# sshaoshuai/PointRCNN

Hardware: AMD Instinct MI355X
Metric: KITTI frames/sec, RPN inference end-to-end (16384 pts/frame, bs32 per GPU) (higher is better)
Workload: dtype f32 via split-bf16x6 MFMA (every fp32 operand cut exactly into 3 bf16 pieces, 6 bf16 MFMA products per fp32 product, fp32 accumulate: fp32-grade, measured error 2.9e-7 of sum|x||w| vs 3.0e-7 for the fp32-MFMA kernel; hoisted grouped layers on the split kernel too, unhoisted grouped first layers (xyz; 1 GPU; Full RPN PointNet++ backbone (4 SA-MSG + 4 FP) + cls/reg heads, tools/cfgs/default.yaml, 16384 pts/frame, batch 32 per GPU, random-init weights, eval-mode BN; frames_per_gpu=32, npoints=16384, parallelism=frames sharded, dp1, launch=hipGraph replay, streams=20, hw_queues=4, proposal_layer=normal, clouds=uniform, group_dedup=True, roi_dedup=True

## Files before the change

### pointrcnn_amd/csrc/fps.hip

```cpp
#include "lds_sort.h"
#include "switches.h"

typedef float f32x2 __attribute__((ext_vector_type(2)));
template <int PPT> struct fvec_t { typedef float type __attribute__((ext_vector_type(PPT))); };
template <> struct fvec_t<1> { typedef float type __attribute__((ext_vector_type(2))); };

#define FPS_DPP_MAX(v, ctrl) asm volatile("s_nop 1\n\tv_max_i32_dpp %0, %0, %0 " ctrl : "+v"(v))

__device__ __forceinline__ int wave_max_i32_fused(int v) {
    FPS_DPP_MAX(v, "row_shr:1 row_mask:0xf bank_mask:0xf");
    FPS_DPP_MAX(v, "row_shr:2 row_mask:0xf bank_mask:0xf");
    FPS_DPP_MAX(v, "row_shr:4 row_mask:0xf bank_mask:0xf");
    FPS_DPP_MAX(v, "row_shr:8 row_mask:0xf bank_mask:0xf");
    FPS_DPP_MAX(v, "row_bcast:15 row_mask:0xa bank_mask:0xf");
    FPS_DPP_MAX(v, "row_bcast:31 row_mask:0xc bank_mask:0xf");
    asm volatile("s_nop 1");
    return __builtin_amdgcn_readlane(v, 63);
}
__device__ __forceinline__ int row0_max_i32_fused(int v) {
    FPS_DPP_MAX(v, "row_shr:1 row_mask:0xf bank_mask:0xf");
    FPS_DPP_MAX(v, "row_shr:2 row_mask:0xf bank_mask:0xf");
    FPS_DPP_MAX(v, "row_shr:4 row_mask:0xf bank_mask:0xf");
    FPS_DPP_MAX(v, "row_shr:8 row_mask:0xf bank_mask:0xf");
    asm volatile("s_nop 1");
// ... 125 lines not shown
        int k = tid * PPT + i;
        bool ok = k < N;
        px[i] = ok ? p[k * 3 + 0] : 0.f;
        py[i] = ok ? p[k * 3 + 1] : 0.f;
        pz[i] = ok ? p[k * 3 + 2] : 0.f;
        pt[i] = ok ? 1e10f : -1.0f;
    }
    if (tid == 0 && npoint > 0) out[0] = 0;
    float x0 = p[0], y0 = p[1], z0 = p[2];

    for (int j = 1; j < npoint; j++) {
        float best = -2.0f;
        if (PPT >= 2) {
            const f32x2 qx = {x0, x0}, qy = {y0, y0}, qz = {z0, z0};
#pragma unroll
            for (int i = 0; i + 1 < PPT; i += 2) {
                f32x2 dx = (f32x2){px[i], px[i + 1]} - qx;
                f32x2 dy = (f32x2){py[i], py[i + 1]} - qy;
                f32x2 dz = (f32x2){pz[i], pz[i + 1]} - qz;
                f32x2 d = (dx * dx + dy * dy) + dz * dz;
                float t0 = __builtin_fminf(pt[i], d.x), t1 = __builtin_fminf(pt[i + 1], d.y);
                pt[i] = t0; pt[i + 1] = t1;
                best = __builtin_fmaxf(best, __builtin_fmaxf(t0, t1));
            }
        } else {
            float d = sqdist3(px[0], py[0], pz[0], x0, y0, z0);
            float t = __builtin_fminf(pt[0], d);
            pt[0] = t;
            best = t;
        }
        const int wmax = wave_max_i32_fused(__float_as_int(best));
        const float wmaxf = __int_as_float(wmax);
        const int owner = __builtin_ctzll(__ballot(best == wmaxf));
        int myslot = PPT - 1;
#pragma unroll
        for (int i = PPT - 2; i >= 0; i--) myslot = (pt[i] == best) ? i : myslot;
        const int istar = __builtin_amdgcn_readlane(myslot, owner);
        const int widx = (wave * 64 + owner) * PPT + istar;
        float sx = px[istar], sy = py[istar], sz = pz[istar];
        float wx = __int_as_float(__builtin_amdgcn_readlane(__float_as_int(sx), owner));
        float wy = __int_as_float(__builtin_amdgcn_readlane(__float_as_int(sy), owner));
        float wz = __int_as_float(__builtin_amdgcn_readlane(__float_as_int(sz), owner));
        int gidx;
        if (NW == 1) {
            gidx = widx; x0 = wx; y0 = wy; z0 = wz;
        } else {
            float* s = slot[j & 1][wave];
            if (lane == 0) {
                s[0] = wmaxf; s[1] = __int_as_float(widx);
                s[2] = wx; s[3] = wy; s[4] = wz;
            }
            __syncthreads();
            const float* r = slot[j & 1][lane < NW ? lane : 0];
            int v = lane < NW ? __float_as_int(r[0]) : (int)0x80000000;
            int id = __float_as_int(r[1]);
            float rx = r[2], ry = r[3], rz = r[4];
            const int gmax = row0_max_i32_fused(v);
            const int wwin = __builtin_ctzll(__ballot(v == gmax));
            gidx = __builtin_amdgcn_readlane(id, wwin);
            x0 = __int_as_float(__builtin_amdgcn_readlane(__float_as_int(rx), wwin));
            y0 = __int_as_float(__builtin_amdgcn_readlane(__float_as_int(ry), wwin));
            z0 = __int_as_float(__builtin_amdgcn_readlane(__float_as_int(rz), wwin));
        }
        if (tid == 0) out[j] = gidx;
    }
}

#define FPS_BIG 1.0e18f
#ifndef FPS_V
#define FPS_V 6
#endif
#ifndef FPS_PAIR_ASM
#define FPS_PAIR_ASM 1
#endif

__device__ __forceinline__ unsigned morton_spread6(unsigned v) {
    v &= 0x3fu;
    v = (v | (v << 8)) & 0x0000300fu;
    v = (v | (v << 4)) & 0x000030c3u;
    v = (v | (v << 2)) & 0x00009249u;
    return v;
}

__global__ __launch_bounds__(1024) void fps_sort_kernel(const float* __restrict__ xyz, int N, int NP, int32_t* __restrict__ perm,
                                                        const int32_t* __restrict__ skip) {
    if (skip && skip[blockIdx.x]) return;
    extern __shared__ unsigned keys[];
    __shared__ float red[6][16];
    const int b = blockIdx.x, tid = threadIdx.x, lane = tid & 63, wave = tid >> 6, nw = blockDim.x >> 6;
    const float* __restrict__ p = xyz + (size_t)b * N * 3;
    float lo[3] = {FPS_BIG, FPS_BIG, FPS_BIG}, hi[3] = {-FPS_BIG, -FPS_BIG, -FPS_BIG};
    for (int k = tid; k < N; k += blockDim.x)
#pragma unroll
        for (int a = 0; a < 3; a++) { float v = p[k * 3 + a]; lo[a] = fminf(lo[a], v); hi[a] = fmaxf(hi[a], v); }
#pragma unroll
    for (int a = 0; a < 3; a++) {
        for (int o = 32; o > 0; o >>= 1) { lo[a] = fminf(lo[a], __shfl_xor(lo[a], o)); hi[a] = fmaxf(hi[a], __shfl_xor(hi[a], o)); }
        if (lane == 0) { red[a][wave] = lo[a]; red[3 + a][wave] = hi[a]; }
    }
    __syncthreads();
    float scale[3];
#pragma unroll
    for (int a = 0; a < 3; a++) {
        float l = red[a][0], h = red[3 + a][0];
        for (int w = 1; w < nw; w++) { l = fminf(l, red[a][w]); h = fmaxf(h, red[3 + a][w]); }
        lo[a] = l;
        scale[a] = (h > l) ? 63.0f / (h - l) : 0.f;
    }
    unsigned v[16];
    if (tid * 16 < NP) {
#pragma unroll
        for (int e = 0; e < 16; e++) {
            const int k = tid * 16 + e;
            unsigned key = ~0u;
            if (k < N) {
                unsigned qx = (unsigned)((p[k * 3 + 0] - lo[0]) * scale[0]);
                unsigned qy = (unsigned)((p[k * 3 + 1] - lo[1]) * scale[1]);
                unsigned qz = (unsigned)((p[k * 3 + 2] - lo[2]) * scale[2]);
                unsigned m = (morton_spread6(qx) << 2) | (morton_spread6(qz) << 1) | morton_spread6(qy);
                key = (m << 14) | (unsigned)k;
            }
            v[e] = key;
        }
    }
    block_sort16(v, keys, NP, tid);
    if (tid * 16 < NP) {
#pragma unroll
        for (int e = 0; e < 16; e++) {
            const int k = tid * 16 + e;
            if (k < N) perm[(size_t)b * N + k] = (int32_t)(v[e] & 0x3fffu);
        }
    }
}

#define FPS_DPP_MIN(v, ctrl) asm volatile("s_nop 1\n\tv_min_i32_dpp %0, %0, %0 " ctrl : "+v"(v))
#define FPS_DPP_FMIN(v, ctrl) asm volatile("s_nop 1\n\tv_min_f32_dpp %0, %0, %0 " ctrl : "+v"(v))
#define FPS_DPP_FMAX(v, ctrl) asm volatile("s_nop 1\n\tv_max_f32_dpp %0, %0, %0 " ctrl : "+v"(v))
#define FPS_WAVE_REDUCE(MACRO, v)                                   \
    MACRO(v, "row_shr:1 row_mask:0xf bank_mask:0xf");               \
    MACRO(v, "row_shr:2 row_mask:0xf bank_mask:0xf");               \
    MACRO(v, "row_shr:4 row_mask:0xf bank_mask:0xf");               \
    MACRO(v, "row_shr:8 row_mask:0xf bank_mask:0xf");               \
    MACRO(v, "row_bcast:15 row_mask:0xa bank_mask:0xf");            \
    MACRO(v, "row_bcast:31 row_mask:0xc bank_mask:0xf");            \
    asm volatile("s_nop 1");

__device__ __forceinline__ int wave_min_i32_fused(int v) { FPS_WAVE_REDUCE(FPS_DPP_MIN, v) return __builtin_amdgcn_readlane(v, 63); }
__device__ __forceinline__ float wave_min_f32_fused(float v) {
    FPS_WAVE_REDUCE(FPS_DPP_FMIN, v) return __int_as_float(__builtin_amdgcn_readlane(__float_as_int(v), 63));
}
__device__ __forceinline__ float wave_max_f32_fused(float v) {
    FPS_WAVE_REDUCE(FPS_DPP_FMAX, v) return __int_as_float(__builtin_amdgcn_readlane(__float_as_int(v), 63));
}
__device__ __forceinline__ int row0_min_i32_fused(int v) {
    FPS_DPP_MIN(v, "row_shr:1 row_mask:0xf bank_mask:0xf");
    FPS_DPP_MIN(v, "row_shr:2 row_mask:0xf bank_mask:0xf");
    FPS_DPP_MIN(v, "row_shr:4 row_mask:0xf bank_mask:0xf");
    FPS_DPP_MIN(v, "row_shr:8 row_mask:0xf bank_mask:0xf");
    asm volatile("s_nop 1");
    return __builtin_amdgcn_readlane(v, 15);
}

#define FPS_XT_DECL __shared__ __attribute__((aligned(256))) unsigned xt[3][64]
struct fps_cand_t { float x, y, z; unsigned long long key; };
__device__ __forceinline__ void fps_cand_set(fps_cand_t& c, int wave, float cx, float cy, float cz, float cval, int corig) {
    const unsigned hi = (unsigned)__float_as_int(cval) ^ 0x80000000u;
    const unsigned lo = ((0xFFFFFFFu - (unsigned)min(corig, 0xFFFFFFF)) << 4) | (unsigned)wave;
    c.x = cx; c.y = cy; c.z = cz; c.key = ((unsigned long long)hi << 32) | lo;
    asm volatile("" : "+v"(c.x), "+v"(c.y), "+v"(c.z), "+v"(c.key));
}
__device__ __forceinline__ void fps_xt_publish(unsigned (*xt)[64], int cb, int wave, const fps_cand_t& c) {
    unsigned* t = xt[cb];
    t[wave] = __float_as_uint(c.x); t[16 + wave] = __float_as_uint(c.y); t[32 + wave] = __float_as_uint(c.z);
    asm volatile("ds_max_u64 %0, %1 offset:192" : : "v"((unsigned)(size_t)&t[0]), "v"(c.key) : "memory");
    if (wave == 0) *(unsigned long long*)&xt[cb == 2 ? 0 : cb + 1][48] = 0ULL;
}
__device__ __forceinline__ int fps_xt_collect(unsigned (*xt)[64], int cb, int lane, float& x0, float& y0, float& z0, int& wl) {
    const int tv = (int)xt[cb][lane];
    const unsigned klo = (unsigned)__builtin_amdgcn_readlane(tv, 48);
    wl = (int)(klo & 15u);
    x0 = __int_as_float(__builtin_amdgcn_readlane(tv, wl));
    y0 = __int_as_float(__builtin_amdgcn_readlane(tv, wl | 16));
    z0 = __int_as_float(__builtin_amdgcn_readlane(tv, wl | 32));
    return (int)(0xFFFFFFFu - (klo >> 4));
}

#ifdef PRCNN_FPS_TIMING
__device__ unsigned long long prcnn_fps_dbg[16 * 8 + 16 + 16 * 16];
PRCNN_API int prcnn_fps_timing_read(unsigned long long* host_out) {
    return hipMemcpyFromSymbol(host_out, HIP_SYMBOL(prcnn_fps_dbg), sizeof(prcnn_fps_dbg)) == hipSuccess ? 0 : -1;
}
#define FPS_T(...) __VA_ARGS__
#ifndef PRCNN_FPS_TIMING_WAVE
#define PRCNN_FPS_TIMING_WAVE -1
#endif
#define FPS_NOW(w) ((PRCNN_FPS_TIMING_WAVE < 0 || (w) == PRCNN_FPS_TIMING_WAVE) ? __builtin_readcyclecounter() : 0ULL)
#else
#define FPS_T(...)
#endif

template <int PPT>
__global__ __launch_bounds__(1024) void fps_pruned_kernel(const float* __restrict__ xyz, const int32_t* __restrict__ perm,
                                                          int N, int npoint, int32_t* __restrict__ idx_out, const int32_t* __restrict__ skip) {
    if (skip && skip[blockIdx.x]) return;
    constexpr int BLOCK = 1024, NW = 16;
    typedef typename fvec_t<PPT>::type fvec;
    FPS_XT_DECL;
    extern __shared__ int s_po[];
// ... 669 lines not shown

__global__ __launch_bounds__(1024) void fps_mem_kernel(const float* __restrict__ xyz, int N, int npoint,
                                                       float* __restrict__ tmp, int32_t* __restrict__ idx_out) {
    constexpr int NW = 16;
    __shared__ int sval[2][NW], sidx[2][NW];
    const int b = blockIdx.x, tid = threadIdx.x, lane = tid & 63, wave = tid >> 6;
    const float* __restrict__ p = xyz + (size_t)b * N * 3;
    float* __restrict__ t = tmp + (size_t)b * N;
    int32_t* __restrict__ out = idx_out + (size_t)b * npoint;
    for (int k = tid; k < N; k += 1024) t[k] = 1e10f;
    if (tid == 0 && npoint > 0) out[0] = 0;
    int old = 0;
    for (int j = 1; j < npoint; j++) {
        float x0 = p[old * 3], y0 = p[old * 3 + 1], z0 = p[old * 3 + 2];
        float best = -2.0f;
        int bk = 0x7fffffff;
        for (int k = tid; k < N; k += 1024) {
            float d = sqdist3(p[k * 3], p[k * 3 + 1], p[k * 3 + 2], x0, y0, z0);
            float v = t[k];
            v = d < v ? d : v;
            t[k] = v;
            if (v > best) { best = v; bk = k; }
        }
        int vb = __float_as_int(best);
        int wmax = wave_max_i32(vb);
        int widx = wave_min_i32(vb == wmax ? bk : 0x7fffffff);
        if (lane == 0) { sval[j & 1][wave] = wmax; sidx[j & 1][wave] = widx; }
        __syncthreads();
        int v = lane < NW ? sval[j & 1][lane] : (int)0x80000000;
        int id = lane < NW ? sidx[j & 1][lane] : 0x7fffffff;
        int gmax = row0_max_i32(v);
        old = row0_min_i32(v == gmax ? id : 0x7fffffff);
        if (tid == 0) out[j] = old;
    }
}

template <int BLOCK, int PPT>
static void launch_fps(const float* xyz, int B, int N, int npoint, int32_t* idx, const int32_t* skip, hipStream_t s) {
    hipLaunchKernelGGL((fps_reg_kernel<BLOCK, PPT>), dim3(B), dim3(BLOCK), 0, s, xyz, N, npoint, idx, skip);
}

static int* fps_timeout_word() {
    static int* word = [] {
        int* w = nullptr;
        if (hipHostMalloc((void**)&w, sizeof(int), hipHostMallocMapped) != hipSuccess) { (void)hipGetLastError(); return (int*)nullptr; }
        *w = 0;
        return w;
    }();
    return word;
}

PRCNN_API int prcnn_fps_status(void) {
    int* w = fps_timeout_word();
    if (w && __atomic_exchange_n(w, 0, __ATOMIC_RELAXED) != 0)
        return prcnn_fail(PRCNN_EHIP, "prcnn_fps: a multi-workgroup launch (N > 16384) gave up waiting for a partner slice; "
                                      "its output holds -1 indices (were all ceil(N/16384) workgroups of a frame able to become resident?)");
    return PRCNN_OK;
}

__global__ __launch_bounds__(256) void fps_prefix_kernel(const float* __restrict__ xyz, const int32_t* __restrict__ prev_idx, int N, int npoint,
                                                         int32_t* __restrict__ idx_out, int32_t* __restrict__ skip) {
    const int b = blockIdx.x, tid = threadIdx.x;
    const float* __restrict__ p = xyz + (size_t)b * N * 3;
    const int32_t* __restrict__ pi = prev_idx + (size_t)b * N;
    int32_t* __restrict__ out = idx_out + (size_t)b * npoint;
    bool ok = true;
    for (int k = tid; k < 3 * N; k += 256) ok &= fabsf(p[k]) < 1e4f;
    for (int j = 1 + tid; j < npoint; j += 256) ok &= pi[j] != 0;
    const int pass = __syncthreads_and(ok) ? 1 : 0;
    if (pass)
        for (int j = tid; j < npoint; j += 256) out[j] = j;
    if (tid == 0) skip[b] = pass;
}

static int fps_dispatch(const float* xyz, int B, int N, int npoint, float* tmp, int32_t* idx, const int32_t* skip, hipStream_t s) {
    if (tmp && N > 2048 && N <= 16384) {
        int NP = 1;
        while (NP < N) NP <<= 1;
        int32_t* perm = reinterpret_cast<int32_t*>(tmp);
        static PrcnnLdsLimit sort_attr;
        if (!sort_attr.raise((const void*)fps_sort_kernel, 80 * 1024))
            return prcnn_fail(PRCNN_EHIP, "prcnn_fps: cannot raise the dynamic LDS limit of the sort kernel");
        const int sort_threads = NP / 16 < 64 ? 64 : NP / 16;
        hipLaunchKernelGGL(fps_sort_kernel, dim3(B), dim3(sort_threads), lds_sort_bytes(NP, sizeof(unsigned)), s, xyz, N, NP, perm, skip);
        PRCNN_LAUNCH_CHECK("prcnn_fps(sort)");
        static PrcnnLdsLimit pruned_attr;
        if (!pruned_attr.raise((const void*)fps_pruned_kernel<16>, 16 * 4096))
            return prcnn_fail(PRCNN_EHIP, "prcnn_fps: cannot raise the dynamic LDS limit of the pruned kernel");
        const bool slots = sw_enabled(SW_FPS_SLOTS);
        static PrcnnLdsLimit slot_attr;
        if (slots && N > 8192 && !slot_attr.raise((const void*)fps_slot_kernel<16, 16>, 16 * 4096))
            return prcnn_fail(PRCNN_EHIP, "prcnn_fps: cannot raise the dynamic LDS limit of the slot kernel");
        const bool batch = sw_opt_in(SW_FPS_BATCH);
        static PrcnnLdsLimit batch_attr;
        if (slots && batch && N > 8192 && !batch_attr.raise((const void*)fps_batch_kernel<16, 16>, 16 * 4096))
            return prcnn_fail(PRCNN_EHIP, "prcnn_fps: cannot raise the dynamic LDS limit of the batch kernel");
        if (slots && batch && N > 8192) hipLaunchKernelGGL((fps_batch_kernel<16, 16>), dim3(B), dim3(1024), 16 * 4096, s, xyz, perm, N, npoint, idx, skip);
        else if (slots && N > 8192) hipLaunchKernelGGL((fps_slot_kernel<16, 16>), dim3(B), dim3(1024), 16 * 4096, s, xyz, perm, N, npoint, idx, skip);
        else if (N <= 4096) hipLaunchKernelGGL((fps_pruned_kernel<4>), dim3(B), dim3(1024), 4 * 4096, s, xyz, perm, N, npoint, idx, skip);
        else if (N <= 8192) hipLaunchKernelGGL((fps_pruned_kernel<8>), dim3(B), dim3(1024), 8 * 4096, s, xyz, perm, N, npoint, idx, skip);
        else hipLaunchKernelGGL((fps_pruned_kernel<16>), dim3(B), dim3(1024), 16 * 4096, s, xyz, perm, N, npoint, idx, skip);
    }
    else if (N <= 64) launch_fps<64, 1>(xyz, B, N, npoint, idx, skip, s);
    else if (N <= 128) launch_fps<64, 2>(xyz, B, N, npoint, idx, skip, s);
    else if (N <= 256) launch_fps<64, 4>(xyz, B, N, npoint, idx, skip, s);
    else if (N <= 512) launch_fps<64, 8>(xyz, B, N, npoint, idx, skip, s);
    else if (N <= 1024) launch_fps<64, 16>(xyz, B, N, npoint, idx, skip, s);
    else if (N <= 2048) launch_fps<256, 8>(xyz, B, N, npoint, idx, skip, s);
    else if (N <= 4096) launch_fps<256, 16>(xyz, B, N, npoint, idx, skip, s);
    else if (N <= 8192) launch_fps<1024, 8>(xyz, B, N, npoint, idx, skip, s);
    else if (N <= 16384) launch_fps<1024, 16>(xyz, B, N, npoint, idx, skip, s);
    else {
        PRCNN_REQUIRE(tmp, "prcnn_fps: N=%d > 16384 needs the (B,N) tmp buffer", N);
        PRCNN_REQUIRE(!skip, "prcnn_fps: the multi-workgroup kernels (N=%d > 16384) take no skip words", N);
        const int S = prcnn_divup(N, FPS_MULTI_SLICE);
        const bool use_mem = sw_present(SW_FPS_MEM);
        if (!use_mem && S <= FPS_MULTI_MAX_SPLIT && ((uintptr_t)tmp & 7) == 0) {
            const size_t slot_bytes = (size_t)B * 2 * S * 5 * sizeof(unsigned long long);
            if (prcnn_fill_words(tmp, 0xFFFFFFFFu, slot_bytes / 4, s) != hipSuccess) return prcnn_fail(PRCNN_EHIP, "prcnn_fps: cannot clear the exchange slots");
            if (int st = prcnn_fps_status()) return st;
            hipLaunchKernelGGL(fps_multi_kernel, dim3(B * S), dim3(1024), 0, s, xyz, N, npoint, S, reinterpret_cast<unsigned long long*>(tmp), idx,
                               fps_timeout_word());
        } else {
            hipLaunchKernelGGL(fps_mem_kernel, dim3(B), dim3(1024), 0, s, xyz, N, npoint, tmp, idx);
        }
    }
    PRCNN_LAUNCH_CHECK("prcnn_fps");
    return PRCNN_OK;
}

PRCNN_API int prcnn_fps(const float* xyz, int B, int N, int npoint, float* tmp, int32_t* idx, prcnn_stream_t stream) {
    PRCNN_REQUIRE(B >= 0 && N > 0 && npoint >= 0, "prcnn_fps: bad shape B=%d N=%d npoint=%d", B, N, npoint);
    PRCNN_REQUIRE(npoint <= N, "prcnn_fps: npoint %d > N %d", npoint, N);
    if (B == 0 || npoint == 0) return PRCNN_OK;
    PRCNN_REQUIRE(xyz && idx, "prcnn_fps: null pointer");
    return fps_dispatch(xyz, B, N, npoint, tmp, idx, nullptr, (hipStream_t)stream);
}

PRCNN_API int prcnn_fps_nested(const float* xyz, const int32_t* prev_idx, int B, int N, int npoint, float* tmp, int32_t* idx, int32_t* skip,
                               prcnn_stream_t stream) {
    PRCNN_REQUIRE(B >= 0 && N > 0 && npoint >= 0, "prcnn_fps_nested: bad shape B=%d N=%d npoint=%d", B, N, npoint);
    PRCNN_REQUIRE(npoint <= N, "prcnn_fps_nested: npoint %d > N %d", npoint, N);
    PRCNN_REQUIRE(N <= 16384, "prcnn_fps_nested: N=%d > 16384 (call prcnn_fps)", N);
    if (B == 0 || npoint == 0) return PRCNN_OK;
    PRCNN_REQUIRE(xyz && prev_idx && idx && skip, "prcnn_fps_nested: null pointer");
    hipStream_t s = (hipStream_t)stream;
    hipLaunchKernelGGL(fps_prefix_kernel, dim3(B), dim3(256), 0, s, xyz, prev_idx, N, npoint, idx, skip);
    PRCNN_LAUNCH_CHECK("prcnn_fps_nested(prefix)");
    return fps_dispatch(xyz, B, N, npoint, tmp, idx, skip, s);
}

__global__ __launch_bounds__(1024) void fps_upstream_order_kernel(const float* __restrict__ xyz, int N, int npoint, int T,
                                                                  float* __restrict__ tmp, int32_t* __restrict__ idx_out) {
    constexpr int NWMAX = 16;
    __shared__ int sval[2][NWMAX], stid[2][NWMAX], sidx[2][NWMAX];
    const int b = blockIdx.x, tid = threadIdx.x, lane = tid & 63, wave = tid >> 6;
    const int nw = (blockDim.x + 63) >> 6;
    const float* __restrict__ p = xyz + (size_t)b * N * 3;
    float* __restrict__ t = tmp + (size_t)b * N;
    int32_t* __restrict__ out = idx_out + (size_t)b * npoint;
    for (int k = tid; k < N; k += blockDim.x) t[k] = 1e10f;
    if (tid == 0 && npoint > 0) out[0] = 0;
    __syncthreads();
    int old = 0;
    for (int j = 1; j < npoint; j++) {
        const float x0 = p[old * 3], y0 = p[old * 3 + 1], z0 = p[old * 3 + 2];
        float best = -2.0f;
// ... 41 lines not shown
```

### pointrcnn_amd/csrc/lds_sort.h

```cpp
#pragma once
#include "common.h"

typedef unsigned long long u64;

__device__ __forceinline__ int lds_phys(int i) { return i + (i >> 4); }

template <class K>
__device__ __forceinline__ void cswap(K& a, K& b, bool up) {
    const bool gt = a > b;
    if (gt == up) { K t = a; a = b; b = t; }
}

template <class K>
__device__ __forceinline__ void merge16(K (&v)[16], bool up) {
#pragma unroll
    for (int j = 8; j >= 1; j >>= 1)
#pragma unroll
        for (int e = 0; e < 16; e++)
            if ((e & j) == 0) cswap(v[e], v[e | j], up);
}

template <class K>
__device__ __forceinline__ void lds_pass(K* keys, int nact, int t, int j, int k) {
    K a[8], c[8];
    if (j <= nact && nact >= 8) {
        const int i0 = ((t & ~(j - 1)) << 1) | (t & (j - 1));
        const int D = 2 * nact, DP = D + (D >> 4);
        K* pa = keys + lds_phys(i0);
        K* pb = keys + lds_phys(i0 + j);
#pragma unroll
        for (int q = 0; q < 8; q++) { a[q] = pa[q * DP]; c[q] = pb[q * DP]; }
#pragma unroll
        for (int q = 0; q < 8; q++) {
            const bool up = ((i0 + q * D) & k) == 0;
            if ((a[q] > c[q]) == up) { pa[q * DP] = c[q]; pb[q * DP] = a[q]; }
        }
    } else {
        int ia[8];
#pragma unroll
        for (int q = 0; q < 8; q++) {
            const int p = q * nact + t;
            ia[q] = ((p & ~(j - 1)) << 1) | (p & (j - 1));
            a[q] = keys[lds_phys(ia[q])]; c[q] = keys[lds_phys(ia[q] + j)];
        }
#pragma unroll
        for (int q = 0; q < 8; q++) {
            const bool up = (ia[q] & k) == 0;
            if ((a[q] > c[q]) == up) { keys[lds_phys(ia[q])] = c[q]; keys[lds_phys(ia[q] + j)] = a[q]; }
        }
    }
}

static inline size_t lds_sort_bytes(int Npad, size_t key_bytes = sizeof(u64)) { return ((size_t)(Npad + (Npad >> 4)) + 1) * key_bytes; }

template <class K>
__device__ __forceinline__ void block_sort16(K (&v)[16], K* keys, int Npad, int t) {
    const int nact = Npad >> 4;
    const bool active = t < nact;
    if (active) {
#pragma unroll
        for (int k = 2; k <= 16; k <<= 1)
#pragma unroll
            for (int j = k >> 1; j >= 1; j >>= 1)
#pragma unroll
                for (int e = 0; e < 16; e++)
                    if ((e & j) == 0) cswap(v[e], v[e | j], k < 16 ? ((e & k) == 0) : ((t & 1) == 0));
#pragma unroll
        for (int e = 0; e < 16; e++) keys[lds_phys(t * 16 + e)] = v[e];
    }
    __syncthreads();
    for (int k = 32; k <= Npad; k <<= 1) {
        for (int j = k >> 1; j >= 16; j >>= 1) {
            if (active) lds_pass(keys, nact, t, j, k);
            __syncthreads();
        }
        if (active) {
#pragma unroll
            for (int e = 0; e < 16; e++) v[e] = keys[lds_phys(t * 16 + e)];
            merge16(v, ((t * 16) & k) == 0);
#pragma unroll
            for (int e = 0; e < 16; e++) keys[lds_phys(t * 16 + e)] = v[e];
        }
        __syncthreads();
    }
}

__device__ __forceinline__ void block_merge16(u64 (&v)[16], u64* keys, int Npad, int t) {
    const int nact = Npad >> 4;
    const bool active = t < nact;
    if (active) {
#pragma unroll
        for (int e = 0; e < 16; e++) keys[lds_phys(t * 16 + e)] = v[e];
    }
    __syncthreads();
    for (int j = Npad >> 1; j >= 16; j >>= 1) {
        if (active) lds_pass(keys, nact, t, j, 1 << 30);
        __syncthreads();
    }
    if (active) {
#pragma unroll
        for (int e = 0; e < 16; e++) v[e] = keys[lds_phys(t * 16 + e)];
        merge16(v, true);
    }
}
```

### pointrcnn_amd/csrc/proposal.hip

```cpp
#include "iou3d_geom.h"
#include "lds_sort.h"
#include "switches.h"

struct DecodeParams {
    const float* roi;
    const float* reg;
    float* out;
    long N;
    int roi_cols, C;
    int nb, nyb, nhb;
    int x_res_l, z_res_l, y_bin_l, y_res_l, y_off, ry_bin_l, ry_res_l, size_l;
    int get_xz_fine, get_y_by_bin, get_ry_fine, y_to_bottom;
    float lbs, half_lbs, scope, lybs, half_lybs, yscope;
    float apc, half_apc, quarter_pi, pi, two_pi;
    float anchor[3];
};

__device__ __forceinline__ int argmax_first(const float* v, int n) {
    int best = 0;
    for (int i = 1; i < n; i++) {
        if (v[best] != v[best]) break;
        if (v[i] > v[best] || v[i] != v[i]) best = i;
    }
    return best;
// ... 27 lines not shown
                }
            }
        }
    } else {
        int r = 0, c = tid;
        while (c >= C) { c -= C; r++; }
        for (int e = tid; e < total; e += DEC_THREADS) {
            rows[r * ld + c] = src[e];
            c += DEC_THREADS;
            while (c >= C) { c -= C; r++; }
        }
    }
    __syncthreads();
    if (lane >= nrows) return;
    const float* rg = rows + lane * ld;
    const float* b = P.roi + (row0 + lane) * P.roi_cols;
    const int xb = argmax_first(rg, P.nb), zb = argmax_first(rg + P.nb, P.nb);
    float px = sub(add(mul((float)xb, P.lbs), P.half_lbs), P.scope);
    float pz = sub(add(mul((float)zb, P.lbs), P.half_lbs), P.scope);
    if (P.get_xz_fine) {
        px = add(px, mul(rg[P.x_res_l + xb], P.lbs));
        pz = add(pz, mul(rg[P.z_res_l + zb], P.lbs));
    }
    float py;
    if (P.get_y_by_bin) {
        int yb = argmax_first(rg + P.y_bin_l, P.nyb);
        float y_res = mul(rg[P.y_res_l + yb], P.lybs);
        py = add(sub(add(mul((float)yb, P.lybs), P.half_lybs), P.yscope), y_res);
        py = add(py, b[1]);
    } else {
        py = add(b[1], rg[P.y_off]);
    }
    const int rb = argmax_first(rg + P.ry_bin_l, P.nhb);
    const float ry_res = mul(rg[P.ry_res_l + rb], P.half_apc);
    float ry;
    if (P.get_ry_fine) {
        ry = sub(add(add(mul((float)rb, P.apc), P.half_apc), ry_res), P.quarter_pi);
    } else {
        float a = add(mul((float)rb, P.apc), ry_res);
        float m = fmodf(a, P.two_pi);
        if (m != 0.0f && m < 0.0f) m = add(m, P.two_pi);
        ry = m > P.pi ? sub(m, P.two_pi) : m;
    }
    const float h = add(mul(rg[P.size_l], P.anchor[0]), P.anchor[0]);
    const float w = add(mul(rg[P.size_l + 1], P.anchor[1]), P.anchor[1]);
    const float l = add(mul(rg[P.size_l + 2], P.anchor[2]), P.anchor[2]);
    if (P.roi_cols == 7) {
        const float ang = -b[6];
        const float ca = (float)cos((double)ang), sa = (float)sin((double)ang);
        const float nx = add(mul(px, ca), mul(pz, -sa));
        const float nz = add(mul(px, sa), mul(pz, ca));
        px = nx; pz = nz;
        ry = add(ry, b[6]);
    }
    px = add(px, b[0]);
    pz = add(pz, b[2]);
    if (P.y_to_bottom) py = add(py, h / 2);
    float* o = P.out + (row0 + lane) * 7;
    o[0] = px; o[1] = py; o[2] = pz; o[3] = h; o[4] = w; o[5] = l; o[6] = ry;
}

#define SPLIT_ALL 0
#define SPLIT_RANGE 1
#define SPLIT_VALID 2

struct SortParams {
    const float* scores;
    const float* boxes3d;
    const uint8_t* valid;
    int32_t* cand;
    int32_t* cnt;
    int N, Npad, mode, nseg, cand_ld;
    int pre1, pre2;
    float r0, r1, r2;
};

__device__ __forceinline__ u64 sort_key(float s, int idx) {
    s = s + 0.0f;
    unsigned u = __float_as_uint(s);
    unsigned ok = (s != s) ? 0xFFFFFFFFu : ((u & 0x80000000u) ? ~u : (u | 0x80000000u));
    return ((u64)(~ok) << 32) | (unsigned)idx;
}

__global__ __launch_bounds__(1024) void sort_split_kernel(SortParams P) {
    extern __shared__ u64 keys[];
    const int b = blockIdx.x, t = threadIdx.x, T = blockDim.x;
    const int N = P.N, Npad = P.Npad;
    const int nact = Npad >> 4;
    const bool active = t < nact;
    unsigned* scratch = (unsigned*)(keys + lds_phys(Npad) + 1);
    u64 v[16];
    if (active) {
        const float* __restrict__ sc = P.scores + (size_t)b * N;
#pragma unroll
        for (int e = 0; e < 16; e++) {
            const int i = t * 16 + e;
            v[e] = i < N ? sort_key(sc[i], i) : ~0ULL;
        }
    }
    block_sort16(v, keys, Npad, t);
    unsigned f1 = 0, f2 = 0;
    int idx[16];
    if (active) {
#pragma unroll
        for (int e = 0; e < 16; e++) {
            const u64 key = v[e];
            idx[e] = (int)(unsigned)key;
            if (key == ~0ULL) { idx[e] = -1; continue; }
            if (P.mode == SPLIT_RANGE) {
                const float z = P.boxes3d[((size_t)b * N + idx[e]) * 7 + 2];
                if (z > P.r0 && z <= P.r1) f1 |= 1u << e;
                if (z > P.r1 && z <= P.r2) f2 |= 1u << e;
            } else if (P.mode == SPLIT_VALID) {
                if (P.valid[(size_t)b * N + idx[e]]) f1 |= 1u << e;
            } else {
                f1 |= 1u << e;
            }
        }
    }
    const unsigned mine = (unsigned)__popc(f1) | ((unsigned)__popc(f2) << 16);
    unsigned inc = mine;
    const int lane = t & 63, wave = t >> 6, nwaves = T >> 6;
#pragma unroll
    for (int d = 1; d < 64; d <<= 1) {
        unsigned o = __shfl_up(inc, d, 64);
        if (lane >= d) inc += o;
    }
    if (lane == 63) scratch[wave] = inc;
    __syncthreads();
    if (wave == 0) {
        unsigned w = lane < nwaves ? scratch[lane] : 0u, winc = w;
#pragma unroll
        for (int d = 1; d < 16; d <<= 1) {
            unsigned o = __shfl_up(winc, d, 64);
            if (lane >= d) winc += o;
        }
        if (lane < nwaves) scratch[16 + lane] = winc - w;
        if (lane == nwaves - 1) scratch[32] = winc;
    }
    __syncthreads();
    const unsigned excl = scratch[16 + wave] + inc - mine;
    const unsigned tot = scratch[32];
    const int n1 = (int)(tot & 0xFFFFu), n2 = (int)(tot >> 16);
    int32_t* c1 = P.cand + (size_t)b * P.nseg * P.cand_ld;
    int32_t* c2 = c1 + P.cand_ld;
    const bool borrow = P.mode == SPLIT_RANGE && n2 == 0;
    if (active) {
        int r1 = (int)(excl & 0xFFFFu), r2 = (int)(excl >> 16);
#pragma unroll
        for (int e = 0; e < 16; e++) {
            if ((f1 >> e) & 1u) {
                if (r1 < P.pre1) c1[r1] = idx[e];
                else if (borrow && r1 - P.pre1 < P.pre2) c2[r1 - P.pre1] = idx[e];
                r1++;
            }
            if ((f2 >> e) & 1u) {
                if (r2 < P.pre2) c2[r2] = idx[e];
                r2++;
            }
        }
    }
    if (t == 0) {
        P.cnt[b * P.nseg] = min(n1, P.pre1);
        if (P.nseg > 1) P.cnt[b * P.nseg + 1] = borrow ? max(0, min(n1 - P.pre1, P.pre2)) : min(n2, P.pre2);
    }
}

#define LARGE_CHUNK 16384
__global__ __launch_bounds__(1024) void large_local_sort_kernel(const float* __restrict__ scores, int N, int Ntot, u64* __restrict__ ws) {
    extern __shared__ u64 keys[];
    const int c = blockIdx.x, b = blockIdx.y, t = threadIdx.x;
    const float* __restrict__ sc = scores + (size_t)b * N;
    const bool desc = c & 1;
    u64 v[16];
#pragma unroll
    for (int e = 0; e < 16; e++) {
        const int i = c * LARGE_CHUNK + t * 16 + e;
        const u64 k = i < N ? sort_key(sc[i], i) : ~0ULL;
        v[e] = desc ? ~k : k;
    }
    block_sort16(v, keys, LARGE_CHUNK, t);
    u64* o = ws + (size_t)b * Ntot + (size_t)c * LARGE_CHUNK + t * 16;
#pragma unroll
    for (int e = 0; e < 16; e++) o[e] = desc ? ~v[e] : v[e];
}
__global__ __launch_bounds__(256) void large_cx_kernel(u64* __restrict__ ws, int Ntot, int j, int k) {
    const int b = blockIdx.y;
    const int p = blockIdx.x * 256 + threadIdx.x;
    if (p >= (Ntot >> 1)) return;
    u64* w = ws + (size_t)b * Ntot;
    const int i = ((p & ~(j - 1)) << 1) | (p & (j - 1));
// ... 533 lines not shown
        if (src >= 0) {
            const float* ib = P.boxes3d + ((size_t)b * P.N + src) * 7;
#pragma unroll
            for (int c = 0; c < 7; c++) ob[c] = ib[c];
            P.out_scores[(size_t)b * P.post + slot] = P.scores[(size_t)b * P.N + src];
        } else {
#pragma unroll
            for (int c = 0; c < 7; c++) ob[c] = 0.0f;
            P.out_scores[(size_t)b * P.post + slot] = 0.0f;
        }
    }
    if (threadIdx.x == 0 && P.out_count) P.out_count[b] = n1 + n2;
}

#define PROPOSAL_MAX_SORT 16384
#define LDS_BUDGET (150 * 1024)

static int pow2_at_least(int n, int lo) {
    int p = lo;
    while (p < n) p <<= 1;
    return p;
}

PRCNN_API int prcnn_decode_bbox_target(const float* roi, int roi_cols, const float* pred_reg, long N, int C, double loc_scope,
                                       double loc_bin_size, int num_head_bin, const float* anchor_size_host, int get_xz_fine,
                                       int get_y_by_bin, double loc_y_scope, double loc_y_bin_size, int get_ry_fine,
                                       int y_to_bottom, float* out, prcnn_stream_t stream) {
    PRCNN_REQUIRE(N >= 0 && C > 0, "prcnn_decode_bbox_target: bad N=%ld C=%d", N, C);
    PRCNN_REQUIRE(roi_cols == 3 || roi_cols == 7, "prcnn_decode_bbox_target: roi_cols must be 3 (xyz) or 7 (boxes), got %d", roi_cols);
    PRCNN_REQUIRE(loc_bin_size > 0 && loc_y_bin_size > 0 && num_head_bin > 0 && anchor_size_host,
                  "prcnn_decode_bbox_target: bad bin configuration");
    DecodeParams P;
    P.nb = (int)(loc_scope / loc_bin_size) * 2;
    P.nyb = (int)(loc_y_scope / loc_y_bin_size) * 2;
    int off = P.nb * 2;
    P.x_res_l = P.nb * 2; P.z_res_l = P.nb * 3;
    if (get_xz_fine) off = P.nb * 4;
    P.y_bin_l = P.y_res_l = P.y_off = 0;
    if (get_y_by_bin) { P.y_bin_l = off; P.y_res_l = off + P.nyb; off += 2 * P.nyb; } else { P.y_off = off; off += 1; }
    P.ry_bin_l = off; P.ry_res_l = off + num_head_bin; P.size_l = off + 2 * num_head_bin;
    PRCNN_REQUIRE(P.nb > 0 && P.size_l + 3 == C, "prcnn_decode_bbox_target: C=%d does not match the bin layout (%d channels expected)",
                  C, P.size_l + 3);
    if (N == 0) return PRCNN_OK;
    PRCNN_REQUIRE(roi && pred_reg && out, "prcnn_decode_bbox_target: null pointer");
    const double PI = 3.141592653589793;
    const double apc = get_ry_fine ? (PI / 2) / num_head_bin : (2 * PI) / num_head_bin;
    P.roi = roi; P.reg = pred_reg; P.out = out; P.N = N; P.roi_cols = roi_cols; P.C = C; P.nhb = num_head_bin;
    P.get_xz_fine = get_xz_fine; P.get_y_by_bin = get_y_by_bin; P.get_ry_fine = get_ry_fine; P.y_to_bottom = y_to_bottom;
    P.lbs = (float)loc_bin_size; P.half_lbs = (float)(loc_bin_size / 2); P.scope = (float)loc_scope;
    P.lybs = (float)loc_y_bin_size; P.half_lybs = (float)(loc_y_bin_size / 2); P.yscope = (float)loc_y_scope;
    P.apc = (float)apc; P.half_apc = (float)(apc / 2); P.quarter_pi = (float)(PI / 4); P.pi = (float)PI; P.two_pi = (float)(2 * PI);
    for (int c = 0; c < 3; c++) P.anchor[c] = anchor_size_host[c];
    const size_t lds = (size_t)64 * (C | 1) * sizeof(float);
    PRCNN_REQUIRE(lds <= 64 * 1024, "prcnn_decode_bbox_target: C=%d too wide", C);
    hipLaunchKernelGGL(decode_kernel, dim3(prcnn_divup(N, 64)), dim3(DEC_THREADS), lds, (hipStream_t)stream, P);
    PRCNN_LAUNCH_CHECK("prcnn_decode_bbox_target");
    return PRCNN_OK;
}

static size_t large_sort_bytes(int B, int N) {
    if (N <= PROPOSAL_MAX_SORT) return 0;
    return (size_t)B * (size_t)pow2_at_least(N, LARGE_CHUNK) * sizeof(u64);
}

static int launch_sort_split(const char* op, SortParams& P, int B, hipStream_t s, u64* large_ws) {
    if (P.N > PROPOSAL_MAX_SORT) {
        const int Ntot = pow2_at_least(P.N, LARGE_CHUNK), nchunks = Ntot / LARGE_CHUNK;
        static PrcnnLdsLimit attr_sort, attr_merge;
        if (!attr_sort.raise((const void*)large_local_sort_kernel, LDS_BUDGET) || !attr_merge.raise((const void*)large_local_merge_kernel, LDS_BUDGET))
            return prcnn_fail(PRCNN_EHIP, "%s: cannot raise the dynamic LDS limit", op);
        const size_t lds = lds_sort_bytes(LARGE_CHUNK);
        hipLaunchKernelGGL(large_local_sort_kernel, dim3(nchunks, B), dim3(1024), lds, s, P.scores, P.N, Ntot, large_ws);
        for (int k = 2 * LARGE_CHUNK; k <= Ntot; k <<= 1) {
            for (int j = k >> 1; j >= LARGE_CHUNK; j >>= 1)
                hipLaunchKernelGGL(large_cx_kernel, dim3(prcnn_divup(Ntot / 2, 256), B), dim3(256), 0, s, large_ws, Ntot, j, k);
            hipLaunchKernelGGL(large_local_merge_kernel, dim3(nchunks, B), dim3(1024), lds, s, large_ws, Ntot, k);
        }
        hipLaunchKernelGGL(large_split_kernel, dim3(B), dim3(1024), 0, s, P, large_ws, Ntot);
        PRCNN_LAUNCH_CHECK(op);
        return PRCNN_OK;
    }
    P.Npad = pow2_at_least(P.N, 16);
    const int threads = max(64, ((P.Npad >> 4) + 63) / 64 * 64);
    const size_t lds = lds_sort_bytes(P.Npad) + 40 * sizeof(unsigned);
    static PrcnnLdsLimit attr_set;
    if (!attr_set.raise((const void*)sort_split_kernel, LDS_BUDGET))
        return prcnn_fail(PRCNN_EHIP, "%s: cannot raise the dynamic LDS limit", op);
    hipLaunchKernelGGL(sort_split_kernel, dim3(B), dim3(threads), lds, s, P);
    PRCNN_LAUNCH_CHECK(op);
    return PRCNN_OK;
}

template <int KIND>
static int launch_greedy_nms_kind(const char* op, const NmsParams& P, int B, hipStream_t s) {
    const size_t lds = greedy_nms_lds_bytes<KIND>(max(P.post1, P.post2));
    if (lds > LDS_BUDGET)
        return prcnn_fail(PRCNN_EUNSUPPORTED, "%s: keeping up to %d boxes needs %zu B of LDS (> %d); use prcnn_nms", op,
                          max(P.post1, P.post2), lds, LDS_BUDGET);
    static PrcnnLdsLimit attr_set;
    if (!attr_set.raise((const void*)greedy_nms_kernel<KIND>, LDS_BUDGET))
        return prcnn_fail(PRCNN_EHIP, "%s: cannot raise the dynamic LDS limit", op);
    hipLaunchKernelGGL(greedy_nms_kernel<KIND>, dim3(P.nseg, B), dim3(NMS_THREADS), lds, s, P);
    PRCNN_LAUNCH_CHECK(op);
    return PRCNN_OK;
}
static int launch_greedy_nms(const char* op, int kind, const NmsParams& P, int B, hipStream_t s) {
    if (kind == PRCNN_NMS_ROTATED) {
        const size_t lds = greedy_nms_rot_lds_bytes(max(P.post1, P.post2));
        if (sw_enabled(SW_NMS_PREFILTER) && lds <= LDS_BUDGET) {
            static PrcnnLdsLimit attr_set;
            if (!attr_set.raise((const void*)greedy_nms_rot_kernel, LDS_BUDGET))
                return prcnn_fail(PRCNN_EHIP, "%s: cannot raise the dynamic LDS limit", op);
            hipLaunchKernelGGL(greedy_nms_rot_kernel, dim3(P.nseg, B), dim3(NMS_RT), lds, s, P);
            PRCNN_LAUNCH_CHECK(op);
            return PRCNN_OK;
        }
        return launch_greedy_nms_kind<PRCNN_NMS_ROTATED>(op, P, B, s);
    }
    {
        const size_t lds = greedy_nms_pre_lds_bytes(max(P.post1, P.post2));
        if (sw_enabled(SW_NMS_PREFILTER) && lds <= LDS_BUDGET) {
            static PrcnnLdsLimit attr_set;
            if (!attr_set.raise((const void*)greedy_nms_pre_kernel, LDS_BUDGET))
                return prcnn_fail(PRCNN_EHIP, "%s: cannot raise the dynamic LDS limit", op);
            hipLaunchKernelGGL(greedy_nms_pre_kernel, dim3(P.nseg, B), dim3(NMS_RT), lds, s, P);
            PRCNN_LAUNCH_CHECK(op);
            return PRCNN_OK;
        }
    }
    return launch_greedy_nms_kind<PRCNN_NMS_NORMAL>(op, P, B, s);
}

static size_t align256(size_t x) { return (x + 255) & ~(size_t)255; }

PRCNN_API size_t prcnn_proposal_workspace_bytes(int B, int N, int pre_max, int post_max) {
    if (B <= 0) return 0;
    return align256((size_t)B * 2 * (size_t)max(pre_max, 1) * 4) + align256((size_t)B * 2 * 4) +
           align256((size_t)B * 2 * (size_t)max(post_max, 1) * 4) + align256((size_t)B * 2 * 4) + align256(large_sort_bytes(B, N));
}

PRCNN_API int prcnn_proposal_layer(const float* scores, const float* boxes3d, int B, int N, int use_range, float r0, float r1,
                                   float r2, int pre1, int pre2, int post1, int post2, float nms_thresh, int nms_kind,
                                   float* out_boxes, float* out_scores, int32_t* out_count, void* workspace,
                                   size_t workspace_bytes, prcnn_stream_t stream) {
    const char* op = "prcnn_proposal_layer";
    PRCNN_REQUIRE(B >= 0 && N >= 0, "%s: bad B=%d N=%d", op, B, N);
    PRCNN_REQUIRE(pre1 >= 0 && pre2 >= 0 && post1 >= 0 && post2 >= 0, "%s: negative top-n", op);
    PRCNN_REQUIRE(nms_kind == PRCNN_NMS_ROTATED || nms_kind == PRCNN_NMS_NORMAL, "%s: bad nms_kind %d", op, nms_kind);
    const int post = post1 + post2;
    if (B == 0 || post == 0) return PRCNN_OK;
    PRCNN_REQUIRE(out_boxes && out_scores, "%s: null output", op);
    hipStream_t s = (hipStream_t)stream;
    if (N == 0) {
        if (prcnn_fill_words(out_boxes, 0u, (size_t)B * post * 7, s) != hipSuccess ||
            prcnn_fill_words(out_scores, 0u, (size_t)B * post, s) != hipSuccess ||
            (out_count && prcnn_fill_words(out_count, 0u, (size_t)B, s) != hipSuccess))
            return prcnn_fail(PRCNN_EHIP, "%s: memset failed", op);
        return PRCNN_OK;
    }
    PRCNN_REQUIRE(scores && boxes3d && workspace, "%s: null pointer", op);
    const int pre_max = max(pre1, pre2), post_max = max(post1, post2);
    PRCNN_REQUIRE(workspace_bytes >= prcnn_proposal_workspace_bytes(B, N, pre_max, post_max), "%s: workspace %zu < %zu bytes", op,
                  workspace_bytes, prcnn_proposal_workspace_bytes(B, N, pre_max, post_max));
    PRCNN_REQUIRE(((uintptr_t)workspace & 7) == 0, "%s: workspace must be 8-byte aligned", op);
    char* w = (char*)workspace;
    int32_t* cand = (int32_t*)w; w += align256((size_t)B * 2 * (size_t)max(pre_max, 1) * 4);
    int32_t* cnt = (int32_t*)w; w += align256((size_t)B * 2 * 4);
// ... 59 lines not shown
```

Baseline: 15120 frames/s.

## Replace bitonic block sorts with LDS radix sort in FPS and proposal split

Adds a block-wide LSD radix sort in LDS. It ranks keys with wave ballots and per-wave digit histograms, then does a block prefix scan. The FPS Morton-key sort (18 key bits, three 6-bit passes) and the proposal score sort (32-bit key with a 16-bit row payload, four 8-bit passes) now use it in place of the bitonic block_sort16. The goal is to cut the compare-exchange work and barriers of the bitonic network. In exchange the code uses more LDS for the histogram tables, relies on a stable sort instead of an index tiebreak in the 64-bit key, and adds many __syncthreads per pass.

```diff
diff --git a/pointrcnn_amd/csrc/fps.hip b/pointrcnn_amd/csrc/fps.hip
--- a/pointrcnn_amd/csrc/fps.hip
+++ b/pointrcnn_amd/csrc/fps.hip
@@ -231,6 +231,9 @@
     return v;
 }
 
+#ifndef FPS_SORT_DIGIT
+#define FPS_SORT_DIGIT 6
+#endif
 __global__ __launch_bounds__(1024) void fps_sort_kernel(const float* __restrict__ xyz, int N, int NP, int32_t* __restrict__ perm,
                                                         const int32_t* __restrict__ skip) {
     if (skip && skip[blockIdx.x]) return;
@@ -272,7 +275,7 @@
             v[e] = key;
         }
     }
-    block_sort16(v, keys, NP, tid);
+    block_radix_sort16<14, 18, FPS_SORT_DIGIT, false>(v, v, keys, nullptr, keys + lds_phys(NP) + 1, N, NP, tid);
     if (tid * 16 < NP) {
 #pragma unroll
         for (int e = 0; e < 16; e++) {
@@ -1108,7 +1111,8 @@
         if (!sort_attr.raise((const void*)fps_sort_kernel, 80 * 1024))
             return prcnn_fail(PRCNN_EHIP, "prcnn_fps: cannot raise the dynamic LDS limit of the sort kernel");
         const int sort_threads = NP / 16 < 64 ? 64 : NP / 16;
-        hipLaunchKernelGGL(fps_sort_kernel, dim3(B), dim3(sort_threads), lds_sort_bytes(NP, sizeof(unsigned)), s, xyz, N, NP, perm, skip);
+        const size_t sort_lds = lds_sort_bytes(NP, sizeof(unsigned)) + radix_tab_words(FPS_SORT_DIGIT, sort_threads) * sizeof(unsigned);
+        hipLaunchKernelGGL(fps_sort_kernel, dim3(B), dim3(sort_threads), sort_lds, s, xyz, N, NP, perm, skip);
         PRCNN_LAUNCH_CHECK("prcnn_fps(sort)");
         static PrcnnLdsLimit pruned_attr;
         if (!pruned_attr.raise((const void*)fps_pruned_kernel<16>, 16 * 4096))
diff --git a/pointrcnn_amd/csrc/lds_sort.h b/pointrcnn_amd/csrc/lds_sort.h
--- a/pointrcnn_amd/csrc/lds_sort.h
+++ b/pointrcnn_amd/csrc/lds_sort.h
@@ -103,3 +103,106 @@
         merge16(v, true);
     }
 }
+
+static inline size_t radix_tab_words(int digit_bits, int threads) { return (size_t)(threads >> 6) * ((1u << digit_bits) + 1) + 16; }
+__host__ __device__ static inline size_t radix_pay_words(int Npad) { return ((size_t)(Npad + (Npad >> 4)) + 2) / 2; }
+
+template <int LO, int NBITS, int DIGIT, bool PAYLOAD>
+__device__ __forceinline__ void block_radix_sort16(unsigned (&v)[16], unsigned (&pl)[16], unsigned* keys, unsigned short* pay, unsigned* tab,
+                                                   int n, int Npad, int t) {
+    static_assert(NBITS % DIGIT == 0 && DIGIT >= 6 && LO + NBITS <= 32, "whole digits of at least 6 bits (one table entry per lane)");
+    constexpr int R = 1 << DIGIT, RS = R + 1, PER = R / 64;
+    const int lane = t & 63, w = t >> 6, W = blockDim.x >> 6, lw = 31 - __clz(W);
+    unsigned* mine = tab + w * RS;
+    unsigned* wsum = tab + W * RS;
+    const int seg = w * 1024 + lane;
+    if (t * 16 < n) {
+#pragma unroll
+        for (int e = 0; e < 16; e++) {
+            keys[lds_phys(t * 16 + e)] = v[e];
+            if (PAYLOAD) pay[lds_phys(t * 16 + e)] = (unsigned short)pl[e];
+        }
+    }
+    __syncthreads();
+#pragma unroll 1
+    for (int shift = LO; shift < LO + NBITS; shift += DIGIT) {
+        unsigned r[16];
+        for (int d = lane; d < R; d += 64) mine[d] = 0;
+#pragma unroll
+        for (int e = 0; e < 16; e++) {
+            const int pos = seg + 64 * e;
+            if (pos < n) {
+                v[e] = keys[lds_phys(pos)];
+                if (PAYLOAD) pl[e] = pay[lds_phys(pos)];
+            }
+        }
+        __builtin_amdgcn_fence(__ATOMIC_ACQ_REL, "wavefront");
+        __syncthreads();
+#pragma unroll
+        for (int e = 0; e < 16; e++) {
+            if (seg + 64 * e < n) {
+                const unsigned d = (v[e] >> shift) & (R - 1);
+                const u64 live = __ballot(1);
+                unsigned dlo = 0, dhi = 0;
+#pragma unroll
+                for (int bit = 0; bit < DIGIT; bit++) {
+                    unsigned ext = (unsigned)((int)(d << (31 - bit)) >> 31);
+                    asm volatile("" : "+v"(ext));
+                    const u64 m = __ballot(ext != 0);
+                    dlo = __builtin_amdgcn_bitop3_b32((unsigned)m, ext, dlo, 0xBE);
+                    dhi = __builtin_amdgcn_bitop3_b32((unsigned)(m >> 32), ext, dhi, 0xBE);
+                }
+                const unsigned plo = ~dlo & (unsigned)live, phi = ~dhi & (unsigned)(live >> 32);
+                const unsigned below = __builtin_amdgcn_mbcnt_hi(phi, __builtin_amdgcn_mbcnt_lo(plo, 0u));
+                const unsigned cnt = (unsigned)(__popc(plo) + __popc(phi));
+                if (below == 0) atomicAdd(&mine[d], cnt);
+                __builtin_amdgcn_fence(__ATOMIC_ACQ_REL, "wavefront");
+                r[e] = mine[d] - cnt + below;
+            }
+            __builtin_amdgcn_fence(__ATOMIC_ACQ_REL, "wavefront");
+        }
+        __syncthreads();
+        unsigned c[PER], sum = 0;
+#pragma unroll
+        for (int q = 0; q < PER; q++) {
+            const int j = t * PER + q;
+            c[q] = tab[(j & (W - 1)) * RS + (j >> lw)];
+            sum += c[q];
+        }
+        unsigned inc = sum;
+#pragma unroll
+        for (int o = 1; o < 64; o <<= 1) {
+            const unsigned up = __shfl_up(inc, o, 64);
+            if (lane >= o) inc += up;
+        }
+        if (lane == 63) wsum[w] = inc;
+        __syncthreads();
+        unsigned run = inc - sum;
+        for (int ww = 0; ww < w; ww++) run += wsum[ww];
+#pragma unroll
+        for (int q = 0; q < PER; q++) {
+            const int j = t * PER + q;
+            tab[(j & (W - 1)) * RS + (j >> lw)] = run;
+            run += c[q];
+        }
+        __syncthreads();
+#pragma unroll
+        for (int e = 0; e < 16; e++) {
+            if (seg + 64 * e < n) {
+                const unsigned d = (v[e] >> shift) & (R - 1);
+                const int dst = lds_phys((int)(mine[d] + r[e]));
+                keys[dst] = v[e];
+                if (PAYLOAD) pay[dst] = (unsigned short)pl[e];
+            }
+        }
+        __syncthreads();
+    }
+    if (t * 16 < Npad) {
+#pragma unroll
+        for (int e = 0; e < 16; e++) {
+            const int pos = t * 16 + e;
+            v[e] = pos < n ? keys[lds_phys(pos)] : ~0u;
+            if (PAYLOAD) pl[e] = pos < n ? (unsigned)pay[lds_phys(pos)] : 0xFFFFu;
+        }
+    }
+}
diff --git a/pointrcnn_amd/csrc/proposal.hip b/pointrcnn_amd/csrc/proposal.hip
--- a/pointrcnn_amd/csrc/proposal.hip
+++ b/pointrcnn_amd/csrc/proposal.hip
@@ -133,31 +133,37 @@
     return ((u64)(~ok) << 32) | (unsigned)idx;
 }
 
+#define SPLIT_DIGIT 8
+static inline size_t sort_split_lds_words(int Npad, int threads) {
+    return (size_t)(Npad + (Npad >> 4)) + 1 + radix_pay_words(Npad) + 40 + radix_tab_words(SPLIT_DIGIT, threads);
+}
+
 __global__ __launch_bounds__(1024) void sort_split_kernel(SortParams P) {
-    extern __shared__ u64 keys[];
+    extern __shared__ unsigned skeys[];
     const int b = blockIdx.x, t = threadIdx.x, T = blockDim.x;
     const int N = P.N, Npad = P.Npad;
     const int nact = Npad >> 4;
     const bool active = t < nact;
-    unsigned* scratch = (unsigned*)(keys + lds_phys(Npad) + 1);
-    u64 v[16];
+    unsigned short* pay = (unsigned short*)(skeys + lds_phys(Npad) + 1);
+    unsigned* scratch = skeys + lds_phys(Npad) + 1 + radix_pay_words(Npad);
+    unsigned v[16], row[16];
     if (active) {
         const float* __restrict__ sc = P.scores + (size_t)b * N;
 #pragma unroll
         for (int e = 0; e < 16; e++) {
             const int i = t * 16 + e;
-            v[e] = i < N ? sort_key(sc[i], i) : ~0ULL;
-        }
-    }
-    block_sort16(v, keys, Npad, t);
+            v[e] = i < N ? (unsigned)(sort_key(sc[i], i) >> 32) : ~0u;
+            row[e] = (unsigned)i;
+        }
+    }
+    block_radix_sort16<0, 32, SPLIT_DIGIT, true>(v, row, skeys, pay, scratch + 40, N, Npad, t);
     unsigned f1 = 0, f2 = 0;
     int idx[16];
     if (active) {
 #pragma unroll
         for (int e = 0; e < 16; e++) {
-            const u64 key = v[e];
-            idx[e] = (int)(unsigned)key;
-            if (key == ~0ULL) { idx[e] = -1; continue; }
+            idx[e] = (int)row[e];
+            if (t * 16 + e >= N) { idx[e] = -1; continue; }
             if (P.mode == SPLIT_RANGE) {
                 const float z = P.boxes3d[((size_t)b * N + idx[e]) * 7 + 2];
                 if (z > P.r0 && z <= P.r1) f1 |= 1u << e;
@@ -857,7 +863,7 @@
     }
     P.Npad = pow2_at_least(P.N, 16);
     const int threads = max(64, ((P.Npad >> 4) + 63) / 64 * 64);
-    const size_t lds = lds_sort_bytes(P.Npad) + 40 * sizeof(unsigned);
+    const size_t lds = sort_split_lds_words(P.Npad, threads) * sizeof(unsigned);
     static PrcnnLdsLimit attr_set;
     if (!attr_set.raise((const void*)sort_split_kernel, LDS_BUDGET))
         return prcnn_fail(PRCNN_EHIP, "%s: cannot raise the dynamic LDS limit", op);
```

Result: no change. 15130 frames/s (median of 2 runs) (+0.1%).
